# DakeQQ/Text-to-Speech-TTS-ONNX

Measured on AMD Instinct MI355X. Metric: audio_seconds_per_second, higher is better.
Workload: dtype f32

## Files before the change

### text-to-speech-tts-onnx_amd/csrc/gemm_epilogue.h

```cpp
#pragma once
#include "common.h"
#include <type_traits>
#include "mfma.h"
#include "x3_split.h"
#include "wave_reduce.h"

namespace mi {

__device__ __forceinline__ float act_apply(float v, int act) {
    switch (act) {
        case ACT_GELU_TANH: {
            const float k0 = 0.7978845608028654f, k1 = 0.044715f;
            return 0.5f * v * (1.f + tanhf(k0 * (v + k1 * v * v * v)));
        }
        case ACT_GELU_ERF: return 0.5f * v * (1.f + erff(v * 0.7071067811865476f));
        case ACT_MISH: {
            float sp = v > 20.f ? v : log1pf(expf(v));
            return v * tanhf(sp);
        }
        case ACT_SILU: return v / (1.f + expf(-v));
        default: return v;
    }
}

// ... 116 lines not shown
                long row = m;
                o = nok && m < p.M;
                if (p.epi == EPI_CONVT) { row = (long)m * p.u + ph - p.padT; o = o && row >= 0 && row < p.T_out; }
                return (o ? row : 0) * p.out_rstride + col;
            };
            auto live = [&](int r) -> bool { return mb + (r & 3) + 8 * (r >> 2) < mlim; };
#pragma unroll
            for (int r = 0; r < 16; ++r) v[r] = acc[i][j][r] + bv;
            switch (p.act) {
                case ACT_GELU_TANH: act16<ACT_GELU_TANH, sizeof(TO) == 2>(v); break;
                case ACT_GELU_ERF: act16<ACT_GELU_ERF>(v); break;
                case ACT_MISH: act16<ACT_MISH>(v); break;
                case ACT_SILU: act16<ACT_SILU>(v); break;
                default: break;
            }
#pragma unroll
            for (int r = 0; r < 16; ++r) v[r] *= gv;
            if (resp) {
#pragma unroll
                for (int r = 0; r < 16; ++r) {
                    bool o; const long ix = row_of(r, o);
                    if constexpr (LENS) o = o && live(r);
                    v[r] += o ? to_f32(resp[ix]) : 0.f;
                }
            }
#pragma unroll
            for (int r = 0; r < 16; ++r) v[r] *= p.alpha;
            if (p.accumulate) {
#pragma unroll
                for (int r = 0; r < 16; ++r) {
                    bool o; const long ix = row_of(r, o);
                    if constexpr (LENS) o = o && live(r);
                    v[r] += o ? to_f32(outp[ix]) : 0.f;
                }
            }
            if constexpr (LENS) {
#pragma unroll
                for (int r = 0; r < 16; ++r) if (!live(r)) v[r] = 0.f;
            }
#pragma unroll
            for (int r = 0; r < 16; ++r) { bool o; const long ix = row_of(r, o); if (o) outp[ix] = from_f32<TO>(v[r]); }
            __builtin_amdgcn_sched_barrier(0);
        }
    }
}

__device__ __forceinline__ int gemm_live_rows(const ConvGemmDev& p, int b) {
    return __builtin_amdgcn_readfirstlane(p.lens[b] * p.len_mul + p.len_add);
}
__device__ __forceinline__ bool gemm_tile_dead(const ConvGemmDev& p, int m0, int vb) {
    return (p.epi == EPI_CONVT ? m0 * p.u - p.padT : m0) >= vb;
}

template <typename TO, int TM, int TN, int WM, int WN>
__device__ __forceinline__ void gemm_epilogue_lds(f32x16 (&acc)[TM][TN], const ConvGemmDev& p, int m0, int n0, int b, int g,
                                                  int wm, int wn, int lr, int lk, float* stage, int m_end = -1) {
    const int Mlim = m_end >= 0 ? m_end : p.M;
    constexpr int CH = sizeof(TO) == 2 ? 8 : 4;
    constexpr int LPR = WN / CH;
    constexpr int RPI = 64 / LPR;
    constexpr int RT = (WN <= 64 && TM % 2 == 0) ? 2 : 1;
    const int lane = lk * 32 + lr;
    TO* outp = (TO*)p.out + (long)b * p.out_bstride;
    const TO* resp = p.res ? (const TO*)p.res + (long)b * p.out_bstride : nullptr;
    const int cl = (lane % LPR) * CH, rl0 = lane / LPR;
    const int nchunk = n0 + wn * WN + cl;
    int ccol = g * p.N + nchunk, cph = 0;
    if (p.epi == EPI_CONVT) { cph = nchunk / p.Cout; ccol = nchunk - cph * p.Cout; }
    const bool cok = nchunk < p.N && lane < RPI * LPR;
#pragma unroll
    for (int i0 = 0; i0 < TM; i0 += RT) {
#pragma unroll
        for (int j = 0; j < TN; ++j) {
            const int n = n0 + wn * WN + j * 32 + lr;
            const int nc = n < p.N ? n : 0;
            const int col = p.epi == EPI_CONVT ? nc % p.Cout : g * p.N + nc;
            const float bv = p.bias ? p.bias[col] : 0.f;
            const float gv = p.gate ? p.gate[(long)b * p.gate_bstride + col] : 1.f;
#pragma unroll
            for (int ii = 0; ii < RT; ++ii) {
                float v[16];
#pragma unroll
                for (int r = 0; r < 16; ++r) v[r] = acc[i0 + ii][j][r] + bv;
                switch (p.act) {
                    case ACT_GELU_TANH: act16<ACT_GELU_TANH, sizeof(TO) == 2>(v); break;
                    case ACT_GELU_ERF: act16<ACT_GELU_ERF>(v); break;
                    case ACT_MISH: act16<ACT_MISH>(v); break;
                    case ACT_SILU: act16<ACT_SILU>(v); break;
                    default: break;
                }
#pragma unroll
                for (int r = 0; r < 16; ++r)
                    stage[(ii * 32 + (r & 3) + 8 * (r >> 2) + 4 * lk) * WN + j * 32 + lr] = v[r] * gv;
            }
        }
        __builtin_amdgcn_fence(__ATOMIC_RELEASE, "wavefront");
        __builtin_amdgcn_wave_barrier();
        constexpr int NIT = (RT * 32 + RPI - 1) / RPI, GRP = NIT % 4 == 0 ? 4 : (NIT % 2 == 0 ? 2 : 1);
        struct alignas(16) Pk { TO v[CH]; };
#pragma unroll
        for (int it0 = 0; it0 < NIT; it0 += GRP) {
            Pk rv[GRP], ov[GRP];
            long ixv[GRP];
            bool okv[GRP];
#pragma unroll
            for (int gi = 0; gi < GRP; ++gi) {
                const int rr = rl0 + (it0 + gi) * RPI;
                const int m = m0 + wm * WM + i0 * 32 + rr;
                long row = m;
                bool ok = cok && rr < RT * 32 && m < Mlim;
                if (p.epi == EPI_CONVT) { row = (long)m * p.u + cph - p.padT; ok = ok && row >= 0 && row < p.T_out; }
                okv[gi] = ok;
                ixv[gi] = ok ? row * p.out_rstride + ccol : 0;
            }
            if (resp) {
#pragma unroll
                for (int gi = 0; gi < GRP; ++gi) rv[gi] = *reinterpret_cast<const Pk*>(resp + ixv[gi]);
            }
            if (p.accumulate) {
#pragma unroll
                for (int gi = 0; gi < GRP; ++gi) ov[gi] = *reinterpret_cast<const Pk*>(outp + ixv[gi]);
            }
#pragma unroll
            for (int gi = 0; gi < GRP; ++gi) {
                const int rr = min(rl0 + (it0 + gi) * RPI, RT * 32 - 1);
                float x[CH];
#pragma unroll
                for (int q = 0; q < CH; q += 4) {
                    const float4 t = *reinterpret_cast<const float4*>(&stage[rr * WN + cl + q]);
                    x[q] = t.x; x[q + 1] = t.y; x[q + 2] = t.z; x[q + 3] = t.w;
                }
                if (resp) {
#pragma unroll
                    for (int q = 0; q < CH; ++q) x[q] += to_f32(rv[gi].v[q]);
                }
#pragma unroll
                for (int q = 0; q < CH; ++q) x[q] *= p.alpha;
                if (p.accumulate) {
#pragma unroll
                    for (int q = 0; q < CH; ++q) x[q] += to_f32(ov[gi].v[q]);
                }
                Pk o;
#pragma unroll
                for (int q = 0; q < CH; ++q) o.v[q] = from_f32<TO>(x[q]);
                if (okv[gi]) *reinterpret_cast<Pk*>(outp + ixv[gi]) = o;
            }
        }
        __builtin_amdgcn_fence(__ATOMIC_ACQUIRE, "wavefront");
        __builtin_amdgcn_wave_barrier();
    }
}


__device__ __forceinline__ void ln_rows32(const ConvGemmDev& p, long row0, long row_last, int lr, int lk, float& rstd, float& mrstd) {
    const int nb = p.ln_dim / LN_BLK;
    long row = row0 + lr;
    row = row < row_last ? row : row_last;
    if (p.ln_final) {
        const float2 t = reinterpret_cast<const float2*>(p.ln_stats_in)[row];
        rstd = t.x; mrstd = t.y;
        return;
    }
    const float* rowp = p.ln_stats_in + row * (long)(nb * 2);
    const float m0 = rowp[0] * (1.0f / 32.0f);
    const float4* sp = reinterpret_cast<const float4*>(rowp) + lk * (nb >> 2);
    LnMerge t;
    for (int i = 0; i < (nb >> 2); ++i) {
        const float4 v = sp[i];
        ln_merge_add(t, v.x, v.y, m0);
        ln_merge_add(t, v.z, v.w, m0);
    }
    LnMerge o;
    o.a = __shfl_xor(t.a, 32); o.b = __shfl_xor(t.b, 32); o.c = __shfl_xor(t.c, 32);
    if (lk) ln_merge_finish(o, t, m0, nb, p.ln_eps, rstd, mrstd);
    else ln_merge_finish(t, o, m0, nb, p.ln_eps, rstd, mrstd);
}

template <typename TO, int TMQ = 2, bool LN = false, bool PRE = false>
__device__ __forceinline__ void gemm_epilogue_qkv_lds(f32x16 (&acc)[TMQ][2], const ConvGemmDev& p, int m0, int n0, int b,
                                                      int wm, int wn, int lr, int lk, float* stage,
                                                      const float* pre_rs = nullptr, const float* pre_mr = nullptr, int m_end = -1) {
    const int Mlim = m_end >= 0 ? m_end : p.M;
    const int lane = lk * 32 + lr;
    const int dm = p.heads * 64;
    const int nbase = n0 + wn * 64;
    const int which = nbase / dm, hh = (nbase - which * dm) >> 6;
    const int Mb = p.Mb > 0 ? p.Mb : p.M;
    const int mrow = m0 + wm * (32 * TMQ);
    const int mbase = mrow + p.m_off;
    const int bi0 = mbase / Mb, mloc0 = mbase - bi0 * Mb;
    const bool vt = which == 2 && p.v_ld > 0;
    TO* base = (TO*)(which == 0 ? p.out : which == 1 ? p.out2 : p.out3);
    struct alignas(16) Pk { TO v[8]; };
    unsigned qkv_sat = 0;
    float ln_rs[TMQ], ln_mr[TMQ];
    if constexpr (LN) {
#pragma unroll
        for (int i = 0; i < TMQ; ++i) {
            if constexpr (PRE) { ln_rs[i] = pre_rs[i]; ln_mr[i] = pre_mr[i]; }
            else ln_rows32(p, (long)mbase + i * 32, (long)p.m_off + p.M - 1, lr, lk, ln_rs[i], ln_mr[i]);
        }
    }
    if (!vt) {
        float ln_pv[8], ln_cv[8];
        if constexpr (LN) {
            const int cc = nbase + (lane & 7) * 8;
            const float4 a0 = *reinterpret_cast<const float4*>(p.ln_p + cc), a1 = *reinterpret_cast<const float4*>(p.ln_p + cc + 4);
            const float4 b0 = *reinterpret_cast<const float4*>(p.ln_c + cc), b1 = *reinterpret_cast<const float4*>(p.ln_c + cc + 4);
            ln_pv[0] = a0.x; ln_pv[1] = a0.y; ln_pv[2] = a0.z; ln_pv[3] = a0.w; ln_pv[4] = a1.x; ln_pv[5] = a1.y; ln_pv[6] = a1.z; ln_pv[7] = a1.w;
            ln_cv[0] = b0.x; ln_cv[1] = b0.y; ln_cv[2] = b0.z; ln_cv[3] = b0.w; ln_cv[4] = b1.x; ln_cv[5] = b1.y; ln_cv[6] = b1.z; ln_cv[7] = b1.w;
        }
#pragma unroll
        for (int j = 0; j < 2; ++j) {
            const float bv = (!LN && p.bias) ? p.bias[nbase + j * 32 + lr] : 0.f;
#pragma unroll
            for (int i = 0; i < TMQ; ++i)
#pragma unroll
                for (int r = 0; r < 16; ++r)
                    stage[(i * 32 + (r & 3) + 8 * (r >> 2) + 4 * lk) * 64 + j * 32 + lr] = acc[i][j][r] + bv;
        }
        __builtin_amdgcn_fence(__ATOMIC_RELEASE, "wavefront");
        __builtin_amdgcn_wave_barrier();
        const int c8 = (lane & 7) * 8;
        struct alignas(16) H8 { f16 v[8]; };
        constexpr int GRP = 4;
#pragma unroll
        for (int it0 = 0; it0 < 4 * TMQ; it0 += GRP) {
            int mv[GRP], biv[GRP];
            bool okv[GRP];
            H8 cs[GRP];
#pragma unroll
            for (int gi = 0; gi < GRP; ++gi) {
                const int rr = (lane >> 3) + (it0 + gi) * 8;
                okv[gi] = mrow + rr < Mlim;
                int m = mloc0 + rr, bi = bi0;
                if (m >= Mb) { m -= Mb; ++bi; }
                if (!okv[gi]) { m = 0; bi = bi0; }
                mv[gi] = m; biv[gi] = bi;
            }
            if (which < 2 && p.rope_pack) {
#pragma unroll
                for (int gi = 0; gi < GRP; ++gi) cs[gi] = *reinterpret_cast<const H8*>((const f16*)p.rope_pack + (long)mv[gi] * 64 + c8);
            }
#pragma unroll
            for (int gi = 0; gi < GRP; ++gi) {
                const int rr = (lane >> 3) + (it0 + gi) * 8;
                float x[8];
#pragma unroll
                for (int q = 0; q < 8; q += 4) {
                    const float4 t = *reinterpret_cast<const float4*>(&stage[rr * 64 + c8 + q]);
                    x[q] = t.x; x[q + 1] = t.y; x[q + 2] = t.z; x[q + 3] = t.w;
                }
                if constexpr (LN) {
                    const float rs = __shfl(ln_rs[(it0 + gi) >> 2], rr & 31), mr = __shfl(ln_mr[(it0 + gi) >> 2], rr & 31);
#pragma unroll
                    for (int q = 0; q < 8; ++q) x[q] = __builtin_fmaf(rs, x[q], __builtin_fmaf(-mr, ln_pv[q], ln_cv[q]));
                }
                if (which < 2 && p.rope_pack) {
#pragma unroll
                    for (int q = 0; q < 8; q += 2) {
                        const float cc = (float)cs[gi].v[q], ss = (float)cs[gi].v[q + 1];
                        const float e = x[q], o = x[q + 1];
                        x[q] = e * cc - o * ss;
                        x[q + 1] = o * cc + e * ss;
                    }
                } else if (which < 2) {
                    float c[8], sn[8];
#pragma unroll
                    for (int q = 0; q < 8; q += 4) {
                        const float4 tc = *reinterpret_cast<const float4*>(p.rope_cos + (long)mv[gi] * 64 + c8 + q);
                        const float4 ts = *reinterpret_cast<const float4*>(p.rope_sin + (long)mv[gi] * 64 + c8 + q);
                        c[q] = tc.x; c[q + 1] = tc.y; c[q + 2] = tc.z; c[q + 3] = tc.w;
                        sn[q] = ts.x; sn[q + 1] = ts.y; sn[q + 2] = ts.z; sn[q + 3] = ts.w;
                    }
#pragma unroll
                    for (int q = 0; q < 8; q += 2) {
                        const float e = x[q], o = x[q + 1];
                        x[q] = e * c[q] - o * sn[q];
                        x[q + 1] = o * c[q + 1] + e * sn[q + 1];
                    }
                }
                if constexpr (sizeof(TO) == 4) if (p.kv_planes && which == 1) {
                    if (p.kv_planes == 2) {
                        x3_u4 pl[2];
                        {
                            unsigned wh[4], wl[4];
#pragma unroll
                            for (int q = 0; q < 4; ++q) x2u_split_pair(x[2 * q], x[2 * q + 1], wh[q], wl[q]);
                            pl[0] = x3_u4{wh[0], wh[1], wh[2], wh[3]}; pl[1] = x3_u4{wl[0], wl[1], wl[2], wl[3]};
                            qkv_sat |= x2_sat_word(wh[0]) | x2_sat_word(wh[1]) | x2_sat_word(wh[2]) | x2_sat_word(wh[3]);
                        }
                        bf16* kp = (bf16*)p.out2 + ((((long)b + biv[gi]) * p.heads + hh) * 2 * p.k_ld + mv[gi]) * 64 + c8;
                        if (okv[gi]) {
                            *reinterpret_cast<x3_u4*>(kp) = pl[0];
                            *reinterpret_cast<x3_u4*>(kp + p.k_ld * 64) = pl[1];
                        }
                        continue;
                    }
                    unsigned p1[4], p2[4], p3[4];
#pragma unroll
                    for (int q = 0; q < 4; ++q) x3_split_pair(x[2 * q], x[2 * q + 1], p1[q], p2[q], p3[q]);
                    bf16* kp = (bf16*)p.out2 + ((((long)b + biv[gi]) * p.heads + hh) * 3 * p.k_ld + mv[gi]) * 64 + c8;
                    if (okv[gi]) {
                        *reinterpret_cast<x3_u4*>(kp) = x3_u4{p1[0], p1[1], p1[2], p1[3]};
                        *reinterpret_cast<x3_u4*>(kp + p.k_ld * 64) = x3_u4{p2[0], p2[1], p2[2], p2[3]};
                        *reinterpret_cast<x3_u4*>(kp + 2 * p.k_ld * 64) = x3_u4{p3[0], p3[1], p3[2], p3[3]};
                    }
                    continue;
                }
                if constexpr (sizeof(TO) == 4) if (p.kv_planes == 2 && which == 0) {
#pragma unroll
                    for (int q = 0; q < 8; ++q) qkv_sat |= (fabsf(x[q]) * 1.4426950408889634f >= 65504.f || x[q] != x[q]) ? 1u : 0u;
                }
                Pk o8;
#pragma unroll
                for (int q = 0; q < 8; ++q) o8.v[q] = from_f32<TO>(x[q]);
                if (okv[gi]) *reinterpret_cast<Pk*>(base + (((long)b + biv[gi]) * p.heads + hh) * Mb * 64 + (long)mv[gi] * 64 + c8) = o8;
            }
        }
        __builtin_amdgcn_fence(__ATOMIC_ACQUIRE, "wavefront");
        __builtin_amdgcn_wave_barrier();
    } else {
        const int row = lane & 31, dh = lane >> 5;
        float ln_pl = 0.f, ln_cl = 0.f;
        if constexpr (LN) { ln_pl = p.ln_p[nbase + lane]; ln_cl = p.ln_c[nbase + lane]; }
#pragma unroll
        for (int i = 0; i < TMQ; ++i) {
#pragma unroll
            for (int j = 0; j < 2; ++j) {
                const float bv = (!LN && p.bias) ? p.bias[nbase + j * 32 + lr] : 0.f;
#pragma unroll
                for (int r = 0; r < 16; ++r)
                    stage[((r & 3) + 8 * (r >> 2) + 4 * lk) * 65 + j * 32 + lr] = acc[i][j][r] + bv;
            }
            auto vt_val = [&](int dd) __attribute__((always_inline)) -> float {
                const float a = stage[row * 65 + dd];
                if constexpr (LN) return __builtin_fmaf(ln_rs[i], a, __builtin_fmaf(-ln_mr[i], __shfl(ln_pl, dd), __shfl(ln_cl, dd)));
                else return a;
            };
            __builtin_amdgcn_fence(__ATOMIC_RELEASE, "wavefront");
            __builtin_amdgcn_wave_barrier();
            const int rr = i * 32 + row;
            const bool ok = mrow + rr < Mlim;
            int m = mloc0 + rr, bi = bi0;
            if (m >= Mb) { m -= Mb; ++bi; }
            TO* dst = base + (((long)b + bi) * p.heads + hh) * 64 * p.v_ld + m;
            if (sizeof(TO) == 4 && p.kv_planes) {
                const long pstride = 64 * p.v_ld;
                if (p.kv_planes == 2) {
                    unsigned short* vp = (unsigned short*)p.out3 + (((long)b + bi) * p.heads + hh) * 2 * 64 * p.v_ld + m;
#pragma unroll 8
                    for (int d = 0; d < 32; ++d) {
                        const int dd = dh * 32 + d;
                        unsigned ph, pl;
                        x2u_split_pair(vt_val(dd), 0.f, ph, pl);
                        qkv_sat |= x2_sat_word(ph);
                        if (ok) {
                            vp[(long)dd * p.v_ld] = (unsigned short)ph;
                            vp[pstride + (long)dd * p.v_ld] = (unsigned short)pl;
                        }
                    }
                } else {
                unsigned short* vp = (unsigned short*)p.out3 + (((long)b + bi) * p.heads + hh) * 3 * 64 * p.v_ld + m;
#pragma unroll 8
                for (int d = 0; d < 32; ++d) {
                    const int dd = dh * 32 + d;
                    unsigned p1, p2, p3;
                    x3_split_pair(vt_val(dd), 0.f, p1, p2, p3);
                    if (ok) {
                        vp[(long)dd * p.v_ld] = (unsigned short)p1;
                        vp[pstride + (long)dd * p.v_ld] = (unsigned short)p2;
                        vp[2 * pstride + (long)dd * p.v_ld] = (unsigned short)p3;
                    }
                }
                }
            } else {
#pragma unroll 8
                for (int d = 0; d < 32; ++d) {
                    const int dd = dh * 32 + d;
                    const float v = vt_val(dd);
                    if (ok) dst[(long)dd * p.v_ld] = from_f32<TO>(v);
                }
            }
            __builtin_amdgcn_fence(__ATOMIC_ACQUIRE, "wavefront");
            __builtin_amdgcn_wave_barrier();
        }
    }
    if constexpr (sizeof(TO) == 4) sat_publish(p.sat, qkv_sat);
}


template <typename TO> __device__ __forceinline__ void ln_act8(float (&x)[8], int act) {
    switch (act) {
        case ACT_GELU_TANH:
#pragma unroll
            for (int q = 0; q < 8; ++q) x[q] = gelu_tanh_fast(x[q]);
            break;
        case ACT_GELU_ERF:
#pragma unroll
            for (int q = 0; q < 8; ++q) x[q] = act_apply(x[q], ACT_GELU_ERF);
            break;
        case ACT_MISH:
#pragma unroll
            for (int q = 0; q < 8; ++q) x[q] = act_apply(x[q], ACT_MISH);
            break;
        case ACT_SILU:
#pragma unroll
            for (int q = 0; q < 8; ++q) x[q] = act_apply(x[q], ACT_SILU);
            break;
        default: break;
    }
}

template <typename TO, int TM, int TN, int NP, bool PRE = false>
__device__ __forceinline__ void gemm_epilogue_ln_in(f32x16 (&acc)[TM][TN], const ConvGemmDev& p, int mw, int nc0, int lr, int lk, float* stage,
                                                    const float* pre_rs = nullptr, const float* pre_mr = nullptr, int m_end = -1) {
    const int Mlim = m_end >= 0 ? m_end : p.M;
    constexpr int WN = 32 * TN, LPR = WN / 8, RPI = 64 / LPR, NIT = 32 / RPI;
    const int lane = lk * 32 + lr;
    const int c8 = (lane % LPR) * 8, rl0 = lane / LPR;
    const int col = nc0 + c8;
    float pv[8], cv[8];
    {
        const float4 a0 = *reinterpret_cast<const float4*>(p.ln_p + col), a1 = *reinterpret_cast<const float4*>(p.ln_p + col + 4);
        const float4 b0 = *reinterpret_cast<const float4*>(p.ln_c + col), b1 = *reinterpret_cast<const float4*>(p.ln_c + col + 4);
        pv[0] = a0.x; pv[1] = a0.y; pv[2] = a0.z; pv[3] = a0.w; pv[4] = a1.x; pv[5] = a1.y; pv[6] = a1.z; pv[7] = a1.w;
        cv[0] = b0.x; cv[1] = b0.y; cv[2] = b0.z; cv[3] = b0.w; cv[4] = b1.x; cv[5] = b1.y; cv[6] = b1.z; cv[7] = b1.w;
    }
    unsigned sat = 0;
    struct alignas(16) Pk { TO v[8]; };
    float rs_all[TM], mr_all[TM];
#pragma unroll
    for (int i = 0; i < TM; ++i) {
        if constexpr (PRE) { rs_all[i] = pre_rs[i]; mr_all[i] = pre_mr[i]; }
        else ln_rows32(p, (long)mw + i * 32, (long)p.M - 1, lr, lk, rs_all[i], mr_all[i]);
    }
#pragma unroll
    for (int i = 0; i < TM; ++i) {
        const float rstd = rs_all[i], mrstd = mr_all[i];
#pragma unroll
        for (int j = 0; j < TN; ++j)
#pragma unroll
            for (int r = 0; r < 16; ++r) stage[((r & 3) + 8 * (r >> 2) + 4 * lk) * WN + j * 32 + lr] = acc[i][j][r];
        __builtin_amdgcn_fence(__ATOMIC_RELEASE, "wavefront");
        __builtin_amdgcn_wave_barrier();
#pragma unroll
        for (int it = 0; it < NIT; ++it) {
            const int rr = rl0 + it * RPI;
            const int m = mw + i * 32 + rr;
            const float rs = __shfl(rstd, rr), mr = __shfl(mrstd, rr);
            const float4 t0 = *reinterpret_cast<const float4*>(&stage[rr * WN + c8]);
            const float4 t1 = *reinterpret_cast<const float4*>(&stage[rr * WN + c8 + 4]);
            float x[8] = {t0.x, t0.y, t0.z, t0.w, t1.x, t1.y, t1.z, t1.w};
#pragma unroll
            for (int q = 0; q < 8; ++q) x[q] = __builtin_fmaf(rs, x[q], __builtin_fmaf(-mr, pv[q], cv[q]));
            ln_act8<TO>(x, p.act);
            if constexpr (sizeof(TO) == 4) {
                x3_u4 pl[NP];
                xnp_split8_sat<NP>(x, pl, sat);
                if (m < Mlim) {
                    unsigned char* dst = (unsigned char*)p.out_planes + x3p_slot_offset(m, col >> 3, p.N >> 5, NP);
#pragma unroll
                    for (int q = 0; q < NP; ++q) *reinterpret_cast<x3_u4*>(dst + q * X3P_PLANE) = pl[q];
                }
            } else {
                Pk o;
#pragma unroll
                for (int q = 0; q < 8; ++q) o.v[q] = from_f32<TO>(x[q]);
                if (m < Mlim) *reinterpret_cast<Pk*>((TO*)p.out + (long)m * p.out_rstride + col) = o;
            }
        }
        __builtin_amdgcn_fence(__ATOMIC_ACQUIRE, "wavefront");
        __builtin_amdgcn_wave_barrier();
    }
    if constexpr (sizeof(TO) == 4 && NP == 2) sat_publish(p.sat, sat);
}

template <typename TA, int TM, int TN, int NP>
__device__ __forceinline__ void gemm_epilogue_resid_ln(f32x16 (&acc)[TM][TN], const ConvGemmDev& p, int mw, int nc0, int lr, int lk, float* stage, int m_end = -1) {
    const int Mlim = m_end >= 0 ? m_end : p.M;
    constexpr int WN = 32 * TN, LPR = WN / 8, RPI = 64 / LPR, NIT = 32 / RPI;
    const int lane = lk * 32 + lr;
    const int c8 = (lane % LPR) * 8, rl0 = lane / LPR;
    const int col = nc0 + c8;
    const int nb = p.N / LN_BLK;
    float* outp = (float*)p.out;
    const float* resp = (const float*)p.res;
    float gsc[8];
    {
        const float4 a0 = *reinterpret_cast<const float4*>(p.ln_scale + col), a1 = *reinterpret_cast<const float4*>(p.ln_scale + col + 4);
        gsc[0] = 1.f + a0.x; gsc[1] = 1.f + a0.y; gsc[2] = 1.f + a0.z; gsc[3] = 1.f + a0.w;
        gsc[4] = 1.f + a1.x; gsc[5] = 1.f + a1.y; gsc[6] = 1.f + a1.z; gsc[7] = 1.f + a1.w;
    }
    unsigned sat = 0;
    struct alignas(16) Pk { TA v[8]; };
#pragma unroll
    for (int i = 0; i < TM; ++i) {
#pragma unroll
        for (int j = 0; j < TN; ++j) {
            const int n = nc0 + j * 32 + lr;
            const float bv = p.bias ? p.bias[n] : 0.f;
            const float gv = p.gate ? p.gate[n] : 1.f;
#pragma unroll
            for (int r = 0; r < 16; ++r) stage[((r & 3) + 8 * (r >> 2) + 4 * lk) * WN + j * 32 + lr] = (acc[i][j][r] + bv) * gv;
        }
        __builtin_amdgcn_fence(__ATOMIC_RELEASE, "wavefront");
        __builtin_amdgcn_wave_barrier();
        float4 r0[NIT], r1[NIT];
        long ix[NIT];
        bool ok[NIT];
#pragma unroll
        for (int it = 0; it < NIT; ++it) {
            const int m = mw + i * 32 + rl0 + it * RPI;
            ok[it] = m < Mlim;
            ix[it] = ok[it] ? (long)m * p.out_rstride + col : 0;
            r0[it] = *reinterpret_cast<const float4*>(resp + ix[it]);
            r1[it] = *reinterpret_cast<const float4*>(resp + ix[it] + 4);
        }
#pragma unroll
        for (int it = 0; it < NIT; ++it) {
            const int rr = rl0 + it * RPI;
            const int m = mw + i * 32 + rr;
            const float4 t0 = *reinterpret_cast<const float4*>(&stage[rr * WN + c8]);
            const float4 t1 = *reinterpret_cast<const float4*>(&stage[rr * WN + c8 + 4]);
            float x[8] = {t0.x + r0[it].x, t0.y + r0[it].y, t0.z + r0[it].z, t0.w + r0[it].w,
                          t1.x + r1[it].x, t1.y + r1[it].y, t1.z + r1[it].z, t1.w + r1[it].w};
            if (ok[it]) {
                *reinterpret_cast<float4*>(outp + ix[it]) = make_float4(x[0], x[1], x[2], x[3]);
                *reinterpret_cast<float4*>(outp + ix[it] + 4) = make_float4(x[4], x[5], x[6], x[7]);
            }
            float s1, s2;
            ln_block_stats(x, s1, s2);
            if (ok[it] && (lane & 3) == 0)
                *reinterpret_cast<float2*>(p.ln_stats_out + ((long)m * nb + (col >> 5)) * 2) = make_float2(s1, s2);
#pragma unroll
            for (int q = 0; q < 8; ++q) x[q] *= gsc[q];
            if constexpr (sizeof(TA) == 4) {
                x3_u4 pl[NP];
                xnp_split8_sat<NP>(x, pl, sat);
                if (ok[it]) {
                    unsigned char* dst = (unsigned char*)p.ln_out + x3p_slot_offset(m, col >> 3, p.N >> 5, NP);
#pragma unroll
                    for (int q = 0; q < NP; ++q) *reinterpret_cast<x3_u4*>(dst + q * X3P_PLANE) = pl[q];
                }
            } else {
                Pk o;
#pragma unroll
                for (int q = 0; q < 8; ++q) o.v[q] = from_f32<TA>(x[q]);
                if (ok[it]) *reinterpret_cast<Pk*>((TA*)p.ln_out + (long)m * p.N + col) = o;
                if constexpr (std::is_same<TA, f16>::value) sat |= ok[it] ? f16_range_word(x) : 0u;
            }
        }
        __builtin_amdgcn_fence(__ATOMIC_ACQUIRE, "wavefront");
        __builtin_amdgcn_wave_barrier();
    }
    if constexpr ((sizeof(TA) == 4 && NP == 2) || std::is_same<TA, f16>::value) sat_publish(p.sat, sat);
}

template <int TM, int TN, int NP>
__device__ __forceinline__ void x3p_epilogue_planes(f32x16 (&acc)[TM][TN], const ConvGemmDev& p, int m0, int n0, int wm, int wn,
                                                    int lr, int lk, float* stage, int m_end = -1) {
    const int Mlim = m_end >= 0 ? m_end : p.M;
    const int lane = lk * 32 + lr;
#pragma unroll
    for (int j = 0; j < TN; ++j) {
        const float bv = p.bias ? p.bias[n0 + wn * 64 + j * 32 + lr] : 0.f;
#pragma unroll
        for (int i = 0; i < TM; ++i) {
            float v[16];
#pragma unroll
            for (int r = 0; r < 16; ++r) v[r] = acc[i][j][r] + bv;
            switch (p.act) {
                case ACT_GELU_TANH: act16<ACT_GELU_TANH, true>(v); break;
                case ACT_GELU_ERF: act16<ACT_GELU_ERF>(v); break;
                case ACT_MISH: act16<ACT_MISH>(v); break;
                case ACT_SILU: act16<ACT_SILU>(v); break;
                default: break;
            }
#pragma unroll
            for (int r = 0; r < 16; ++r) stage[(i * 32 + (r & 3) + 8 * (r >> 2) + 4 * lk) * 64 + j * 32 + lr] = v[r];
        }
    }
    __builtin_amdgcn_fence(__ATOMIC_RELEASE, "wavefront");
    __builtin_amdgcn_wave_barrier();
    const int nch_out = p.N >> 5;
    const int c8 = (lane & 7) * 8;
    const int s8 = (n0 + wn * 64 + c8) >> 3;
    unsigned char* planes = (unsigned char*)p.out_planes;
    unsigned sat = 0;
#pragma unroll
    for (int it = 0; it < 4 * TM; ++it) {
        const int rr = (lane >> 3) + it * 8;
        const int m = m0 + wm * (32 * TM) + rr;
        const float4 t0 = *reinterpret_cast<const float4*>(&stage[rr * 64 + c8]);
        const float4 t1 = *reinterpret_cast<const float4*>(&stage[rr * 64 + c8 + 4]);
        const float v[8] = {t0.x, t0.y, t0.z, t0.w, t1.x, t1.y, t1.z, t1.w};
        x3_u4 pl[NP];
        xnp_split8_sat<NP>(v, pl, sat);
        if (m < Mlim) {
            unsigned char* dst = planes + x3p_slot_offset(m, s8, nch_out, NP);
#pragma unroll
            for (int q = 0; q < NP; ++q) *reinterpret_cast<x3_u4*>(dst + q * X3P_PLANE) = pl[q];
        }
    }
    __builtin_amdgcn_fence(__ATOMIC_ACQUIRE, "wavefront");
    __builtin_amdgcn_wave_barrier();
    if constexpr (NP == 2) sat_publish(p.sat, sat);
}

typedef __attribute__((address_space(3))) void lds_void;

template <typename T, typename TO> void launch_conv_gemm_dma3(const ConvGemmDev& e, int bn, hipStream_t s);
template <typename T, typename TO> void launch_linear_sk(const ConvGemmDev& e, int stages, hipStream_t s);
void launch_linear_x3(const ConvGemmDev& e, hipStream_t s);
template <typename T, typename TO> void launch_linear_ph8(const ConvGemmDev& e, hipStream_t s);
void launch_linear_x3p(const ConvGemmDev& e, hipStream_t s);
bool x3d_plan(const ConvGemmDev& e, int cus, int& tw, int& rgn, int& cgn, int& band);
void launch_linear_x3d(const ConvGemmDev& e, int tw, int rgn, int cgn, int band, hipStream_t s);


}
```

### text-to-speech-tts-onnx_amd/csrc/gemm_x3d.hip

```cpp
#include "common.h"
#include "mfma.h"
#include "gemm_epilogue.h"
#include "x3_split.h"
#include <type_traits>
#include <algorithm>

namespace mi {

typedef float f32x4 __attribute__((ext_vector_type(4)));

template <int TW> struct X3dGeom {
    static constexpr int TM = 144, MB = 3;
    static constexpr int KG = TW == 64 ? 2 : 1;
    static constexpr int WNS = KG == 2 ? 2 : 4;
    static constexpr int WNW = TW / WNS, NB = WNW / 16;
#ifndef X3D_S128
#define X3D_S128 1
#endif
    static constexpr int S = TW == 192 ? 1 : TW == 128 ? X3D_S128 : 2;
    static constexpr int WSTEP = TW == 128 ? X3D_S128 : 1;
    static constexpr int R = TW == 64 ? 6 : TW == 128 ? 4 : 3;
    static constexpr int LB = R / S - 1;
    static constexpr int A_PLANE = TM * 64, B_PLANE = TW * 64;
    static constexpr int A_BYTES = 2 * A_PLANE, CH = A_BYTES + 2 * B_PLANE;
    static constexpr int PC = CH / 1024, P = S * PC;
    static constexpr int NHI = (P + 11) / 12, NHIW = P - 12 * (NHI - 1);
    static constexpr int NCB = TW / 64, NRB = 5, BLK = 2176;
    static constexpr int STG = NRB * NCB * BLK * 4, RING = R * CH;
    static constexpr int LNT = RING > STG ? RING : STG;
    static constexpr int SMEM = LNT + 2 * 160 * 4;
    static_assert(SMEM <= 163840, "x3d: LDS");
};

template <typename RSRC>
__device__ __forceinline__ void x3d_dma(RSRC rsrc, int voff, unsigned lds_dst) {
#if defined(__HIP_DEVICE_COMPILE__)
    unsigned keep;
    asm volatile("s_mov_b32 %0, m0\n\ts_mov_b32 m0, %3\n\ts_nop 0\n\tbuffer_load_dwordx4 %1, %2, 0 offen lds\n\ts_mov_b32 m0, %0"
                 : "=&s"(keep) : "v"(voff), "s"(rsrc), "s"(lds_dst) : "memory");
#endif
}
template <int N> __device__ __forceinline__ void x3d_wait_lgkm() {
#if defined(__HIP_DEVICE_COMPILE__)
    asm volatile("s_waitcnt lgkmcnt(%0)" :: "n"(N) : "memory");
#endif
}
template <int OFF> __device__ __forceinline__ void x3d_lds_rd128(f16x8& d, unsigned a) {
#if defined(__HIP_DEVICE_COMPILE__)
    asm volatile("ds_read_b128 %0, %1 offset:%2" : "=v"(d) : "v"(a), "n"(OFF) : "memory");
#endif
}
template <int OFF, int N> struct X3dRd {
    static __device__ __forceinline__ void go(f16x8 (&dst)[N], unsigned a) {
        X3dRd<OFF, N - 1>::go(reinterpret_cast<f16x8 (&)[N - 1]>(dst), a);
        x3d_lds_rd128<OFF + (N - 1) * 1024>(dst[N - 1], a);
    }
};
template <int OFF> struct X3dRd<OFF, 1> {
    static __device__ __forceinline__ void go(f16x8 (&dst)[1], unsigned a) { x3d_lds_rd128<OFF>(dst[0], a); }
};
template <int N, int I = 0, typename F> __device__ __forceinline__ void x3d_unroll(F&& f) {
    if constexpr (I < N) { f(std::integral_constant<int, I>{}); x3d_unroll<N, I + 1>(f); }
}
template <int N> __device__ __forceinline__ void x3d_wait_vm() {
#if defined(__HIP_DEVICE_COMPILE__)
    asm volatile("s_waitcnt vmcnt(%0)" :: "n"(N) : "memory");
#endif
}

template <int TW, bool FOLD, int EPK>
__global__ __launch_bounds__(768) void linear_x3d_kernel(const ConvGemmDev p) {
    using G = X3dGeom<TW>;
    using Frag = f16x8;
    constexpr int MB = G::MB, NB = G::NB;
    __shared__ __attribute__((aligned(1024))) unsigned char smem[G::SMEM];
    (void)smem;
#if defined(__HIP_DEVICE_COMPILE__)
    const int tid = threadIdx.x, lane = tid & 63;
    const int wave = __builtin_amdgcn_readfirstlane(tid >> 6);
    const int per = (int)gridDim.x >> 3;
    const int u = ((int)blockIdx.x & 7) * per + ((int)blockIdx.x >> 3);
    const int RGn = p.Tm, CGn = p.Tn, band = p.RT;
    if (u >= RGn * CGn) return;
    const int bi = u / (band * CGn);
    const int rem = u - bi * band * CGn;
    const int bh = min(band, RGn - bi * band);
    const int cg = rem / bh, rg = bi * band + rem - cg * bh;
    const int m0 = rg * G::TM, n0 = cg * TW;
    const int nch = p.K >> 5;

    const int kg = G::KG == 2 ? wave / 6 : 0;
    const int w6 = G::KG == 2 ? wave - kg * 6 : wave;
    const int wm = w6 / G::WNS, wn = w6 - wm * G::WNS;

    const int bytesA = (int)((long)((p.M + 127) >> 7) * nch * 16384), bytesB = (int)((long)((p.N + 127) >> 7) * nch * 16384);
    const unsigned smem_lds = (unsigned)(unsigned long)(const __attribute__((address_space(3))) void*)smem;
    const int voff = lane * 16;
    constexpr int OOB = 0x7fffff00;
    int pc_gbase[G::NHI], pc_cs[G::NHI];
    unsigned pc_lofs[G::NHI];
    __amdgpu_buffer_rsrc_t pc_rs[G::NHI];
#pragma unroll
    for (int i = 0; i < G::NHI; ++i) {
        const int q = wave + 12 * i;
        const int cs = q / G::PC, r = q - cs * G::PC;
        const bool isA = r < 18;
        const int rr = isA ? r : r - 18;
        const int gpp = isA ? 9 : TW / 16;
        const int plane = rr / gpp, g16 = rr - plane * gpp;
        const int row = (isA ? m0 : n0) + 16 * g16;
        pc_cs[i] = cs;
        pc_rs[i] = __builtin_amdgcn_make_buffer_rsrc(isA ? (void*)p.x : (void*)p.w3, 0, isA ? bytesA : bytesB, 0x00020000);
        pc_gbase[i] = __builtin_amdgcn_readfirstlane((row >> 7) * nch * 16384 + plane * 8192 + (row & 127) * 64);
        pc_lofs[i] = (unsigned)__builtin_amdgcn_readfirstlane(isA ? plane * G::A_PLANE + g16 * 1024 : G::A_BYTES + plane * G::B_PLANE + g16 * 1024);
    }
    const bool hi_wave = wave < G::NHIW;
    auto issue_piece = [&](int t, auto I_) __attribute__((always_inline)) {
        constexpr int i = decltype(I_)::value;
        if constexpr (i < G::NHI) {
            if (i == G::NHI - 1 && !hi_wave) return;
            const int chunk = t * G::S + pc_cs[i];
            const int soff = __builtin_amdgcn_readfirstlane(chunk < nch ? pc_gbase[i] + chunk * 16384 : OOB);
            const unsigned dst = __builtin_amdgcn_readfirstlane(smem_lds + (unsigned)((chunk % G::R) * G::CH) + pc_lofs[i]);
            x3d_dma(pc_rs[i], (int)((unsigned)voff + (unsigned)soff), dst);
        }
    };
    auto issue_batch = [&](int t) __attribute__((always_inline)) {
        x3d_unroll<G::NHI>([&](auto I_) __attribute__((always_inline)) { issue_piece(t, I_); });
    };
    auto wait_batches = [&](auto NB_) __attribute__((always_inline)) {
        constexpr int n = decltype(NB_)::value;
        if (hi_wave) x3d_wait_vm<n * G::NHI>(); else x3d_wait_vm<n * (G::NHI - 1)>();
    };

    const int fi = lane & 15, fs = lane >> 4;
    const int sig = (0x1320 >> (4 * (fi >> 2))) & 3;
    const unsigned f_lane = (unsigned)((4 * sig + (fi & 3)) * 64 + ((fs ^ sig) << 4));
    const unsigned fa_off = (unsigned)(wm * 48 * 64) + f_lane;
    const unsigned fb_off = (unsigned)(G::A_BYTES + wn * G::WNW * 64) + f_lane;
    Frag a_lo[MB], a_hi[MB], b_lo[NB], b_hi[NB];
    f32x4 acc0[MB][NB], acc1[MB][NB];
#pragma unroll
    for (int i = 0; i < MB; ++i)
#pragma unroll
        for (int j = 0; j < NB; ++j) { acc0[i][j] = f32x4{0.f, 0.f, 0.f, 0.f}; acc1[i][j] = f32x4{0.f, 0.f, 0.f, 0.f}; }
    auto rd_a = [&](unsigned a, auto PL, Frag (&dst)[MB]) __attribute__((always_inline)) {
        constexpr int pl = decltype(PL)::value;
        X3dRd<pl * G::A_PLANE, MB>::go(dst, a);
    };
    auto rd_b = [&](unsigned b, auto PL, Frag (&dst)[NB]) __attribute__((always_inline)) {
        constexpr int pl = decltype(PL)::value;
        X3dRd<pl * G::B_PLANE, NB>::go(dst, b);
    };
    using P0 = std::integral_constant<int, 0>;
    using P1 = std::integral_constant<int, 1>;
    auto mma = [&](const Frag (&a)[MB], const Frag (&b)[NB], f32x4 (&c)[MB][NB]) __attribute__((always_inline)) {
#pragma unroll
        for (int i = 0; i < MB; ++i)
#pragma unroll
            for (int j = 0; j < NB; ++j) c[i][j] = __builtin_amdgcn_mfma_f32_16x16x32_f16(a[i], b[j], c[i][j], 0, 0, 0);
    };
#define X3D_SB() __builtin_amdgcn_sched_barrier(0)

    const int NJ = nch / G::KG;
#pragma unroll
    for (int t = 0; t <= G::LB; ++t) issue_batch(t);
    float* lnt = reinterpret_cast<float*>(smem + G::LNT);
    constexpr bool CONSUMER = FOLD && (EPK == 1 || EPK == 2);
    if constexpr (CONSUMER) {
        if (wave < G::NRB && p.ln_stats_in) {
            float rs, mr;
            ln_rows32(p, (long)p.m_off + m0 + wave * 32, (long)p.m_off + p.M - 1, lane & 31, lane >> 5, rs, mr);
            if (lane < 32) { lnt[wave * 32 + lane] = rs; lnt[160 + wave * 32 + lane] = mr; }
        }
    }
    wait_batches(std::integral_constant<int, G::LB>{});
    __builtin_amdgcn_s_barrier();
    {
        const unsigned s0 = smem_lds + (unsigned)((kg % G::R) * G::CH);
        rd_a(s0 + fa_off, P1{}, a_lo); rd_b(s0 + fb_off, P0{}, b_hi); rd_a(s0 + fa_off, P0{}, a_hi); rd_b(s0 + fb_off, P1{}, b_lo);
    }
    auto chunk = [&](int j, auto BAR_) __attribute__((always_inline)) {
        constexpr bool BAR = decltype(BAR_)::value;
        x3d_wait_lgkm<MB + NB>();
        X3D_SB(); mma(a_lo, b_hi, acc1); X3D_SB();
        const int jn = j + 1;
        const int ts = jn / G::WSTEP;
        if constexpr (BAR) {
            wait_batches(std::integral_constant<int, G::LB - 1>{});
            asm volatile("s_waitcnt lgkmcnt(0)" ::: "memory");
            __builtin_amdgcn_s_barrier();
        }
        const unsigned sn = smem_lds + (unsigned)(((jn * G::KG + kg) % G::R) * G::CH);
        rd_a(sn + fa_off, P1{}, a_lo);
        x3d_wait_lgkm<MB>();
        X3D_SB();
        x3d_unroll<MB * NB>([&](auto IDX_) __attribute__((always_inline)) {
            constexpr int idx = decltype(IDX_)::value, i = idx / NB, jj = idx % NB;
            acc0[i][jj] = __builtin_amdgcn_mfma_f32_16x16x32_f16(a_hi[i], b_hi[jj], acc0[i][jj], 0, 0, 0);
            if constexpr (BAR) issue_piece(ts + G::LB, IDX_);
            X3D_SB();
        });
        rd_b(sn + fb_off, P0{}, b_hi);
        X3D_SB(); mma(a_hi, b_lo, acc1); X3D_SB();
        rd_a(sn + fa_off, P0{}, a_hi); rd_b(sn + fb_off, P1{}, b_lo);
    };
    static_assert(G::NHI <= MB * NB, "x3d: a batch's pieces ride on the MFMAs of phase 1");
    for (int j = 0; j < NJ; j += G::WSTEP) {
        if constexpr (G::WSTEP == 2) chunk(j, std::false_type{});
        chunk(j + G::WSTEP - 1, std::true_type{});
    }
#undef X3D_SB
    asm volatile("s_waitcnt vmcnt(0)" ::: "memory");
    asm volatile("s_waitcnt lgkmcnt(0)" ::: "memory");
    __builtin_amdgcn_s_barrier();
    if (p.dbg & 4) return;

    float* stg = reinterpret_cast<float*>(smem);
    {
        const int rq = 4 * ((0x1320 >> (4 * (lane >> 4))) & 3);
        const int cq = 4 * ((0x1320 >> (4 * ((lane & 15) >> 2))) & 3) + (lane & 3);
        auto put = [&](bool add) __attribute__((always_inline)) {
#pragma unroll
            for (int i = 0; i < MB; ++i) {
                const int row = wm * 48 + i * 16 + rq;
#pragma unroll
                for (int j = 0; j < NB; ++j) {
                    const int col = wn * G::WNW + j * 16 + cq;
                    float* d = stg + ((row >> 5) * G::NCB + (col >> 6)) * G::BLK + (row & 31) * 64 + (col & 63);
#pragma unroll
                    for (int r = 0; r < 4; ++r) {
                        const float v = __builtin_fmaf(acc1[i][j][r], 0x1p-11f, acc0[i][j][r]);
                        d[r * 64] = add ? d[r * 64] + v : v;
                    }
                }
            }
        };
        if (G::KG == 1 || kg == 0) put(false);
        __syncthreads();
        if constexpr (G::KG == 2) {
            if (kg == 1) put(true);
            __syncthreads();
        }
    }
    const int lr = lane & 31, lk = lane >> 5;
    const int m_end = min(p.M, m0 + G::TM);
    constexpr bool HALVES = EPK == 3 && (G::NRB * G::NCB * G::BLK + 12 * 1024) * 4 <= G::LNT;
    if constexpr (HALVES) {
        float* half_stage = stg + G::NRB * G::NCB * G::BLK;
        for (int u = wave; u < G::NRB * G::NCB * 2; u += 12) {
            const int b = u >> 1, hf = u & 1;
            const int rb = b / G::NCB, cb = b - rb * G::NCB;
            if (m0 + rb * 32 >= m_end) continue;
            const float* blk = stg + b * G::BLK + hf * 32;
            f32x16 h1[1][1];
#pragma unroll
            for (int r = 0; r < 16; ++r) {
                const float t = blk[((r & 3) + 8 * (r >> 2) + 4 * lk) * 64 + lr];
                h1[0][0][r] = (rb == G::NRB - 1 && r >= 8) ? 0.f : t;
            }
            float* st = half_stage + wave * 1024;
            if constexpr (FOLD) gemm_epilogue_resid_ln<float, 1, 1, 2>(h1, p, m0 + rb * 32, n0 + cb * 64 + hf * 32, lr, lk, st, m_end);
            else gemm_epilogue_lds<float, 1, 1, 32, 32>(h1, p, m0, n0, 0, 0, rb, cb * 2 + hf, lr, lk, st, m_end);
        }
        return;
    }
    for (int b = wave; b < G::NRB * G::NCB; b += 12) {
        const int rb = b / G::NCB, cb = b - rb * G::NCB;
        if (m0 + rb * 32 >= m_end) continue;
        float* blk = stg + b * G::BLK;
        float prs[1] = {0.f}, pmr[1] = {0.f};
        if constexpr (CONSUMER) { prs[0] = lnt[rb * 32 + lr]; pmr[0] = lnt[160 + rb * 32 + lr]; }
        f32x16 h[1][2];
#pragma unroll
        for (int j = 0; j < 2; ++j)
#pragma unroll
            for (int r = 0; r < 16; ++r) {
                const float t = blk[((r & 3) + 8 * (r >> 2) + 4 * lk) * 64 + j * 32 + lr];
                h[0][j][r] = (rb == G::NRB - 1 && r >= 8) ? 0.f : t;
            }
        __builtin_amdgcn_fence(__ATOMIC_ACQUIRE, "wavefront");
        __builtin_amdgcn_wave_barrier();
        if constexpr (FOLD) {
            if constexpr (EPK == 1) gemm_epilogue_qkv_lds<float, 1, true, true>(h, p, m0, n0, 0, rb, cb, lr, lk, blk, prs, pmr, m_end);
            else if constexpr (EPK == 2) gemm_epilogue_ln_in<float, 1, 2, 2, true>(h, p, m0 + rb * 32, n0 + cb * 64, lr, lk, blk, prs, pmr, m_end);
            else gemm_epilogue_resid_ln<float, 1, 2, 2>(h, p, m0 + rb * 32, n0 + cb * 64, lr, lk, blk, m_end);
        } else {
            if constexpr (EPK == 1) gemm_epilogue_qkv_lds<float, 1>(h, p, m0, n0, 0, rb, cb, lr, lk, blk, nullptr, nullptr, m_end);
            else if constexpr (EPK == 2) x3p_epilogue_planes<1, 2, 2>(h, p, m0, n0, rb, cb, lr, lk, blk, m_end);
            else gemm_epilogue_lds<float, 1, 2, 32, 64>(h, p, m0, n0, 0, 0, rb, cb, lr, lk, blk, m_end);
        }
    }
#endif
}


bool x3d_plan(const ConvGemmDev& e, int cus, int& tw, int& rgn, int& cgn, int& band) {
    if (!opt(OPT_GEMM_X3D) || e.np != 2 || !e.lds_epi || e.K % 32 != 0 || cus < 8) return false;
    const int nch = e.K / 32;
    double best = 0.0; int btw = 0;
    for (int w : {192, 128, 64}) {
        if (e.N % w != 0) continue;
        if (w != 192 && nch % 2 != 0) continue;
        if (e.epi == EPI_QKV_ROPE && w % 64 != 0) continue;
        const long tiles = (long)((e.M + 143) / 144) * (e.N / w);
        const long rounds = (tiles + cus - 1) / cus;
        const double eff = (double)e.M * e.N / ((double)rounds * cus * 144.0 * w);
        if (eff > best + 1e-9) { best = eff; btw = w; }
    }
    if (!btw || best * 100.0 < (double)opt(OPT_GEMM_X3D_MIN_EFF)) return false;
    tw = btw; rgn = (e.M + 143) / 144; cgn = e.N / btw;
    int ba = 1; double bc = 1e300;
    for (int a = 1; a <= 32; a *= 2) {
        if (a > rgn && a > 1) break;
        const double c = (double)std::min(a, rgn) * 144.0 + (double)std::min(32 / a, cgn) * tw;
        if (c < bc) { bc = c; ba = a; }
    }
    band = std::min(ba, rgn);
    return true;
}

void launch_linear_x3d(const ConvGemmDev& e_in, int tw, int rgn, int cgn, int band, hipStream_t s) {
    ConvGemmDev e = e_in;
    e.Tm = rgn; e.Tn = cgn; e.RT = band;
    const long tiles = (long)rgn * cgn;
    const dim3 grid((unsigned)(((tiles + 7) / 8) * 8));
    const bool fold = e.ln_stats_in || e.ln_stats_out;
    const int epk = e.epi == EPI_QKV_ROPE ? 1 : fold ? (e.ln_stats_in ? 2 : 3) : (e.out_planes ? 2 : 3);
#define X3D_GO(TW_, FOLD_, EPK_, LABEL)                                                                                           \
    do {                                                                                                                          \
        prof_set_kernel("linear_x3d_kernel<" #TW_ ", " LABEL ">", "", "");                                                        \
        hipLaunchKernelGGL((linear_x3d_kernel<TW_, FOLD_, EPK_>), grid, dim3(768), 0, s, e);                                      \
    } while (0)
#define X3D_ROLE(TW_)                                                                                                             \
    do {                                                                                                                          \
        if (fold) { if (epk == 1) X3D_GO(TW_, true, 1, "AdaLN fold, QKV"); else if (epk == 2) X3D_GO(TW_, true, 2, "AdaLN fold, FF1"); else X3D_GO(TW_, true, 3, "AdaLN fold, O / FF2"); } \
        else { if (epk == 1) X3D_GO(TW_, false, 1, "QKV"); else if (epk == 2) X3D_GO(TW_, false, 2, "planes out"); else X3D_GO(TW_, false, 3, "rows out"); } \
    } while (0)
    if (tw == 192) X3D_ROLE(192); else if (tw == 128) X3D_ROLE(128); else X3D_ROLE(64);
#undef X3D_ROLE
#undef X3D_GO
    MI_HIP(hipGetLastError());
}

}
```

Before: 41.74.

## Add direct per-wave epilogue for AdaLN-folded FF1 and O/FF2 x3d GEMMs

Adds a direct epilogue path to the x3d GEMM kernel for the folded-LN roles. The accumulators are staged once into a padded LDS tile in the dead ring, and each of the 12 waves then processes a balanced set of 8-row by 32-column units. Per-column constants are loaded before the main loop, and residual rows are prefetched early when few iterations are needed. It also wraps the residual and LN arithmetic in helpers with FP contraction disabled, so that results match the staged path bit for bit. The older staged epilogue stays available behind an environment variable, at the cost of an extra kernel instantiation and more register pressure from the preloaded values.

Result: no change. 41.59 (-0.4%).

```diff
diff --git a/text-to-speech-tts-onnx_amd/csrc/gemm_epilogue.h b/text-to-speech-tts-onnx_amd/csrc/gemm_epilogue.h
--- a/text-to-speech-tts-onnx_amd/csrc/gemm_epilogue.h
+++ b/text-to-speech-tts-onnx_amd/csrc/gemm_epilogue.h
@@ -292,6 +292,19 @@
 }
 
 
+__device__ __forceinline__ float resid_gated(float acc, float bias, float gate) {
+#pragma clang fp contract(off)
+    const float s = acc + bias;
+    return s * gate;
+}
+__device__ __forceinline__ float resid_add(float gated, float res) {
+#pragma clang fp contract(off)
+    return gated + res;
+}
+__device__ __forceinline__ float ln_finish(float rstd, float mrstd, float acc, float ln_p, float ln_c) {
+    return __builtin_fmaf(rstd, acc, __builtin_fmaf(-mrstd, ln_p, ln_c));
+}
+
 __device__ __forceinline__ void ln_rows32(const ConvGemmDev& p, long row0, long row_last, int lr, int lk, float& rstd, float& mrstd) {
     const int nb = p.ln_dim / LN_BLK;
     long row = row0 + lr;
@@ -394,7 +407,7 @@
                 if constexpr (LN) {
                     const float rs = __shfl(ln_rs[(it0 + gi) >> 2], rr & 31), mr = __shfl(ln_mr[(it0 + gi) >> 2], rr & 31);
 #pragma unroll
-                    for (int q = 0; q < 8; ++q) x[q] = __builtin_fmaf(rs, x[q], __builtin_fmaf(-mr, ln_pv[q], ln_cv[q]));
+                    for (int q = 0; q < 8; ++q) x[q] = ln_finish(rs, mr, x[q], ln_pv[q], ln_cv[q]);
                 }
                 if (which < 2 && p.rope_pack) {
 #pragma unroll
@@ -475,7 +488,7 @@
             }
             auto vt_val = [&](int dd) __attribute__((always_inline)) -> float {
                 const float a = stage[row * 65 + dd];
-                if constexpr (LN) return __builtin_fmaf(ln_rs[i], a, __builtin_fmaf(-ln_mr[i], __shfl(ln_pl, dd), __shfl(ln_cl, dd)));
+                if constexpr (LN) return ln_finish(ln_rs[i], ln_mr[i], a, __shfl(ln_pl, dd), __shfl(ln_cl, dd));
                 else return a;
             };
             __builtin_amdgcn_fence(__ATOMIC_RELEASE, "wavefront");
@@ -593,7 +606,7 @@
             const float4 t1 = *reinterpret_cast<const float4*>(&stage[rr * WN + c8 + 4]);
             float x[8] = {t0.x, t0.y, t0.z, t0.w, t1.x, t1.y, t1.z, t1.w};
 #pragma unroll
-            for (int q = 0; q < 8; ++q) x[q] = __builtin_fmaf(rs, x[q], __builtin_fmaf(-mr, pv[q], cv[q]));
+            for (int q = 0; q < 8; ++q) x[q] = ln_finish(rs, mr, x[q], pv[q], cv[q]);
             ln_act8<TO>(x, p.act);
             if constexpr (sizeof(TO) == 4) {
                 x3_u4 pl[NP];
@@ -642,7 +655,7 @@
             const float bv = p.bias ? p.bias[n] : 0.f;
             const float gv = p.gate ? p.gate[n] : 1.f;
 #pragma unroll
-            for (int r = 0; r < 16; ++r) stage[((r & 3) + 8 * (r >> 2) + 4 * lk) * WN + j * 32 + lr] = (acc[i][j][r] + bv) * gv;
+            for (int r = 0; r < 16; ++r) stage[((r & 3) + 8 * (r >> 2) + 4 * lk) * WN + j * 32 + lr] = resid_gated(acc[i][j][r], bv, gv);
         }
         __builtin_amdgcn_fence(__ATOMIC_RELEASE, "wavefront");
         __builtin_amdgcn_wave_barrier();
@@ -663,8 +676,8 @@
             const int m = mw + i * 32 + rr;
             const float4 t0 = *reinterpret_cast<const float4*>(&stage[rr * WN + c8]);
             const float4 t1 = *reinterpret_cast<const float4*>(&stage[rr * WN + c8 + 4]);
-            float x[8] = {t0.x + r0[it].x, t0.y + r0[it].y, t0.z + r0[it].z, t0.w + r0[it].w,
-                          t1.x + r1[it].x, t1.y + r1[it].y, t1.z + r1[it].z, t1.w + r1[it].w};
+            float x[8] = {resid_add(t0.x, r0[it].x), resid_add(t0.y, r0[it].y), resid_add(t0.z, r0[it].z), resid_add(t0.w, r0[it].w),
+                          resid_add(t1.x, r1[it].x), resid_add(t1.y, r1[it].y), resid_add(t1.z, r1[it].z), resid_add(t1.w, r1[it].w)};
             if (ok[it]) {
                 *reinterpret_cast<float4*>(outp + ix[it]) = make_float4(x[0], x[1], x[2], x[3]);
                 *reinterpret_cast<float4*>(outp + ix[it] + 4) = make_float4(x[4], x[5], x[6], x[7]);
diff --git a/text-to-speech-tts-onnx_amd/csrc/gemm_x3d.hip b/text-to-speech-tts-onnx_amd/csrc/gemm_x3d.hip
--- a/text-to-speech-tts-onnx_amd/csrc/gemm_x3d.hip
+++ b/text-to-speech-tts-onnx_amd/csrc/gemm_x3d.hip
@@ -32,6 +32,19 @@
     static_assert(SMEM <= 163840, "x3d: LDS");
 };
 
+template <int TW> struct X3dEpi {
+    static constexpr int UR = 8, UC = 32;
+    static constexpr int RU = 144 / UR, UNITS = RU * (TW / UC);
+    static constexpr int UPW = UNITS / 12;
+    static_assert(UNITS % 12 == 0, "x3d: every wave carries exactly the mean number of work units (none is above it)");
+    static_assert(RU % UPW == 0, "x3d: a wave's units are consecutive row octets of ONE column chunk");
+    static constexpr int NIT = (UPW + 1) / 2;
+    static constexpr int LD = TW + 4;
+    static constexpr int TILE = 144 * LD;
+    static_assert(X3dGeom<TW>::KG * TILE * 4 <= X3dGeom<TW>::LNT, "x3d: the staged tile(s) fit the dead ring");
+};
+template <bool FOLD, int EPK> constexpr bool X3D_DIRECT = FOLD && (EPK == 2 || EPK == 3);
+
 template <typename RSRC>
 __device__ __forceinline__ void x3d_dma(RSRC rsrc, int voff, unsigned lds_dst) {
 #if defined(__HIP_DEVICE_COMPILE__)
@@ -68,13 +81,13 @@
 #endif
 }
 
-template <int TW, bool FOLD, int EPK>
-__global__ __launch_bounds__(768) void linear_x3d_kernel(const ConvGemmDev p) {
+template <int TW, bool FOLD, int EPK, bool DIRECT>
+__device__ __forceinline__ void linear_x3d_body(const ConvGemmDev& p, unsigned char* smem) {
     using G = X3dGeom<TW>;
+    using E = X3dEpi<TW>;
     using Frag = f16x8;
     constexpr int MB = G::MB, NB = G::NB;
-    __shared__ __attribute__((aligned(1024))) unsigned char smem[G::SMEM];
-    (void)smem;
+    static_assert(!DIRECT || X3D_DIRECT<FOLD, EPK>, "x3d: no direct epilogue for this role");
 #if defined(__HIP_DEVICE_COMPILE__)
     const int tid = threadIdx.x, lane = tid & 63;
     const int wave = __builtin_amdgcn_readfirstlane(tid >> 6);
@@ -162,6 +175,44 @@
     };
 #define X3D_SB() __builtin_amdgcn_sched_barrier(0)
 
+    const int m_end = min(p.M, m0 + G::TM);
+    const int e_cc = wave * E::UPW / E::RU, e_ro0 = wave * E::UPW - e_cc * E::RU;
+    const int e_col = e_cc * E::UC + (lane & 3) * 8;
+    const int e_row0 = (e_ro0 + (lane >> 5)) * E::UR + ((lane >> 2) & 7);
+    auto e_live = [&](int it) __attribute__((always_inline)) {
+        return (E::UPW % 2 == 0 || it < E::NIT - 1 || lane < 32) && m0 + e_row0 + 16 * it < m_end;
+    };
+    float4 e_c0[2], e_c1[2], e_c2[2];
+    float4 e_res[E::NIT][2];
+    constexpr bool RES_EARLY = E::NIT <= 3;
+    auto e_res_load = [&]() __attribute__((always_inline)) {
+#pragma unroll
+        for (int it = 0; it < E::NIT; ++it) {
+            const float* rp = (const float*)p.res + (e_live(it) ? (long)(m0 + e_row0 + 16 * it) * p.out_rstride + n0 + e_col : 0);
+            e_res[it][0] = *reinterpret_cast<const float4*>(rp);
+            e_res[it][1] = *reinterpret_cast<const float4*>(rp + 4);
+        }
+    };
+    if constexpr (DIRECT) {
+        const int col = n0 + e_col;
+        const float4 zero4 = make_float4(0.f, 0.f, 0.f, 0.f), one4 = make_float4(1.f, 1.f, 1.f, 1.f);
+        if constexpr (EPK == 3) {
+#pragma unroll
+            for (int h = 0; h < 2; ++h) {
+                e_c0[h] = p.bias ? *reinterpret_cast<const float4*>(p.bias + col + 4 * h) : zero4;
+                e_c1[h] = p.gate ? *reinterpret_cast<const float4*>(p.gate + col + 4 * h) : one4;
+                e_c2[h] = *reinterpret_cast<const float4*>(p.ln_scale + col + 4 * h);
+            }
+            if constexpr (RES_EARLY) e_res_load();
+        } else {
+#pragma unroll
+            for (int h = 0; h < 2; ++h) {
+                e_c0[h] = *reinterpret_cast<const float4*>(p.ln_p + col + 4 * h);
+                e_c1[h] = *reinterpret_cast<const float4*>(p.ln_c + col + 4 * h);
+            }
+        }
+    }
+
     const int NJ = nch / G::KG;
 #pragma unroll
     for (int t = 0; t <= G::LB; ++t) issue_batch(t);
@@ -216,6 +267,86 @@
     __builtin_amdgcn_s_barrier();
     if (p.dbg & 4) return;
 
+    if constexpr (DIRECT) {
+        float* stg = reinterpret_cast<float*>(smem);
+        if constexpr (EPK == 3 && !RES_EARLY) e_res_load();
+        {
+            const int rq = 4 * ((0x1320 >> (4 * (lane >> 4))) & 3);
+            const int cq = 4 * ((0x1320 >> (4 * ((lane & 15) >> 2))) & 3) + (lane & 3);
+#pragma unroll
+            for (int i = 0; i < MB; ++i)
+#pragma unroll
+                for (int j = 0; j < NB; ++j) {
+                    float* d = stg + kg * E::TILE + (wm * 48 + i * 16 + rq) * E::LD + wn * G::WNW + j * 16 + cq;
+#pragma unroll
+                    for (int r = 0; r < 4; ++r) d[r * E::LD] = __builtin_fmaf(acc1[i][j][r], 0x1p-11f, acc0[i][j][r]);
+                }
+        }
+        __syncthreads();
+        const int col = n0 + e_col;
+        unsigned sat = 0;
+        float gsc[8];
+        if constexpr (EPK == 3) {
+            gsc[0] = 1.f + e_c2[0].x; gsc[1] = 1.f + e_c2[0].y; gsc[2] = 1.f + e_c2[0].z; gsc[3] = 1.f + e_c2[0].w;
+            gsc[4] = 1.f + e_c2[1].x; gsc[5] = 1.f + e_c2[1].y; gsc[6] = 1.f + e_c2[1].z; gsc[7] = 1.f + e_c2[1].w;
+        }
+        const float c0[8] = {e_c0[0].x, e_c0[0].y, e_c0[0].z, e_c0[0].w, e_c0[1].x, e_c0[1].y, e_c0[1].z, e_c0[1].w};
+        const float c1[8] = {e_c1[0].x, e_c1[0].y, e_c1[0].z, e_c1[0].w, e_c1[1].x, e_c1[1].y, e_c1[1].z, e_c1[1].w};
+#pragma unroll
+        for (int it = 0; it < E::NIT; ++it) {
+            const bool ok = e_live(it);
+            const int row = ok ? e_row0 + 16 * it : 0;
+            const int m = m0 + row;
+            const float* sp = stg + row * E::LD + e_col;
+            float4 t0 = *reinterpret_cast<const float4*>(sp), t1 = *reinterpret_cast<const float4*>(sp + 4);
+            if constexpr (G::KG == 2) {
+                const float4 u0 = *reinterpret_cast<const float4*>(sp + E::TILE), u1 = *reinterpret_cast<const float4*>(sp + E::TILE + 4);
+                t0 = make_float4(t0.x + u0.x, t0.y + u0.y, t0.z + u0.z, t0.w + u0.w);
+                t1 = make_float4(t1.x + u1.x, t1.y + u1.y, t1.z + u1.z, t1.w + u1.w);
+            }
+            float x[8] = {t0.x, t0.y, t0.z, t0.w, t1.x, t1.y, t1.z, t1.w};
+            x3_u4 pl[2];
+            unsigned s_it = 0;
+            if constexpr (EPK == 3) {
+                const float r[8] = {e_res[it][0].x, e_res[it][0].y, e_res[it][0].z, e_res[it][0].w,
+                                    e_res[it][1].x, e_res[it][1].y, e_res[it][1].z, e_res[it][1].w};
+#pragma unroll
+                for (int q = 0; q < 8; ++q) x[q] = resid_add(resid_gated(x[q], c0[q], c1[q]), r[q]);
+                if (ok) {
+                    float* op = (float*)p.out + (long)m * p.out_rstride + col;
+                    *reinterpret_cast<float4*>(op) = make_float4(x[0], x[1], x[2], x[3]);
+                    *reinterpret_cast<float4*>(op + 4) = make_float4(x[4], x[5], x[6], x[7]);
+                }
+                float s1, s2;
+                ln_block_stats(x, s1, s2);
+                if (ok && (lane & 3) == 0)
+                    *reinterpret_cast<float2*>(p.ln_stats_out + ((long)m * (p.N / LN_BLK) + (col >> 5)) * 2) = make_float2(s1, s2);
+#pragma unroll
+                for (int q = 0; q < 8; ++q) x[q] *= gsc[q];
+                xnp_split8_sat<2>(x, pl, s_it);
+                if (ok) {
+                    unsigned char* dst = (unsigned char*)p.ln_out + x3p_slot_offset(m, col >> 3, p.N >> 5, 2);
+                    *reinterpret_cast<x3_u4*>(dst) = pl[0];
+                    *reinterpret_cast<x3_u4*>(dst + X3P_PLANE) = pl[1];
+                }
+            } else {
+                const float rs = lnt[row], mr = lnt[160 + row];
+#pragma unroll
+                for (int q = 0; q < 8; ++q) x[q] = ln_finish(rs, mr, x[q], c0[q], c1[q]);
+                ln_act8<float>(x, p.act);
+                xnp_split8_sat<2>(x, pl, s_it);
+                if (ok) {
+                    unsigned char* dst = (unsigned char*)p.out_planes + x3p_slot_offset(m, col >> 3, p.N >> 5, 2);
+                    *reinterpret_cast<x3_u4*>(dst) = pl[0];
+                    *reinterpret_cast<x3_u4*>(dst + X3P_PLANE) = pl[1];
+                }
+            }
+            sat |= ok ? s_it : 0u;
+        }
+        sat_publish(p.sat, sat);
+        return;
+    }
+
     float* stg = reinterpret_cast<float*>(smem);
     {
         const int rq = 4 * ((0x1320 >> (4 * (lane >> 4))) & 3);
@@ -244,7 +375,6 @@
         }
     }
     const int lr = lane & 31, lk = lane >> 5;
-    const int m_end = min(p.M, m0 + G::TM);
     constexpr bool HALVES = EPK == 3 && (G::NRB * G::NCB * G::BLK + 12 * 1024) * 4 <= G::LNT;
     if constexpr (HALVES) {
         float* half_stage = stg + G::NRB * G::NCB * G::BLK;
@@ -294,6 +424,24 @@
 #endif
 }
 
+template <int TW, bool FOLD, int EPK>
+__global__ __launch_bounds__(768) void linear_x3d_kernel(const ConvGemmDev p) {
+    __shared__ __attribute__((aligned(1024))) unsigned char smem[X3dGeom<TW>::SMEM];
+    linear_x3d_body<TW, FOLD, EPK, X3D_DIRECT<FOLD, EPK>>(p, smem);
+}
+template <int TW, bool FOLD, int EPK>
+__global__ __launch_bounds__(768) void linear_x3d_staged_kernel(const ConvGemmDev p) {
+    __shared__ __attribute__((aligned(1024))) unsigned char smem[X3dGeom<TW>::SMEM];
+    linear_x3d_body<TW, FOLD, EPK, false>(p, smem);
+}
+
+template <int TW, bool FOLD, int EPK>
+static void x3d_go(const ConvGemmDev& e, bool direct, dim3 grid, hipStream_t s) {
+    if constexpr (X3D_DIRECT<FOLD, EPK>) {
+        if (!direct) { hipLaunchKernelGGL((linear_x3d_staged_kernel<TW, FOLD, EPK>), grid, dim3(768), 0, s, e); return; }
+    }
+    hipLaunchKernelGGL((linear_x3d_kernel<TW, FOLD, EPK>), grid, dim3(768), 0, s, e);
+}
 
 bool x3d_plan(const ConvGemmDev& e, int cus, int& tw, int& rgn, int& cgn, int& band) {
     if (!opt(OPT_GEMM_X3D) || e.np != 2 || !e.lds_epi || e.K % 32 != 0 || cus < 8) return false;
@@ -327,10 +475,11 @@
     const dim3 grid((unsigned)(((tiles + 7) / 8) * 8));
     const bool fold = e.ln_stats_in || e.ln_stats_out;
     const int epk = e.epi == EPI_QKV_ROPE ? 1 : fold ? (e.ln_stats_in ? 2 : 3) : (e.out_planes ? 2 : 3);
+    const bool direct = env_int("MI355TTS_X3D_EPI", 1) != 0;
 #define X3D_GO(TW_, FOLD_, EPK_, LABEL)                                                                                           \
     do {                                                                                                                          \
         prof_set_kernel("linear_x3d_kernel<" #TW_ ", " LABEL ">", "", "");                                                        \
-        hipLaunchKernelGGL((linear_x3d_kernel<TW_, FOLD_, EPK_>), grid, dim3(768), 0, s, e);                                      \
+        x3d_go<TW_, FOLD_, EPK_>(e, direct, grid, s);                                                                             \
     } while (0)
 #define X3D_ROLE(TW_)                                                                                                             \
     do {                                                                                                                          \
```
